# UniBwTAS/continuous_clustering

Hardware: AMD Instinct MI355X
Metric: Mpoints/s clustered (64-beam streams) (higher is better)
Workload: dtype f32

## Files before the change

continuous_clustering_amd/csrc/cc_engine.hip:

```cpp
#include <hip/hip_runtime.h>

#include <algorithm>
#include <chrono>
#include <cstdlib>
#include <cmath>
#include <cstdio>
#include <cstring>
#include <functional>
#include <limits>
#include <mutex>
#include <string>
#include <vector>

#include "cc_kernels.h"

#ifndef CC_LWAVE_MAX_STREAMS
#define CC_LWAVE_MAX_STREAMS 256
#endif

using namespace ccd;

struct cc_engine
{
    int device{0};
// ... 1483 lines not shown
    c->is_single_threaded = 0;
    c->sensor_is_clockwise = 1;
    c->num_columns = 1700;
    c->supplement_inclination_angle_for_nan_cells = 1;
    c->max_slope = 0.2f;
    c->first_ring_as_ground_max_allowed_z_diff = 0.4f;
    c->first_ring_as_ground_min_allowed_z_diff = -0.4f;
    c->last_ground_point_slope_higher_than = -0.1f;
    c->last_ground_point_distance_smaller_than = 5.f;
    c->ground_because_close_to_last_certain_ground_max_z_diff = 0.4f;
    c->ground_because_close_to_last_certain_ground_max_dist_diff = 2.0f;
    c->obstacle_because_next_certain_obstacle_max_dist_diff = 0.3f;
    c->use_terrain = 0;
    c->terrain_max_allowed_z_diff = 0.4f;
    c->fog_filtering_enabled = 0;
    c->fog_filtering_intensity_below = 2;
    c->fog_filtering_distance_below = 18.f;
    c->fog_filtering_inclination_above = -0.06f;
    c->max_distance = 0.7f;
    c->max_steps_in_row = 20;
    c->max_steps_in_column = 20;
    c->stop_after_association_enabled = 1;
    c->stop_after_association_min_steps = 1;
    c->ignore_points_in_chessboard_pattern = 1;
    c->ignore_points_with_too_big_inclination_angle_diff = 1;
    c->use_last_point_for_cluster_stamp = 0;
    c->cluster_point_trees_every_nth_column = 1;
}

void cc_config_kitti(cc_config* c)
{
    cc_config_default(c);
    c->is_single_threaded = 1;
    c->num_columns = 2200;
    c->ignore_points_in_chessboard_pattern = 0;
    c->max_distance = 0.5f;
    c->height_ref_to_maximum_ = 0.5f;
    c->height_ref_to_ground_ = -1.7f;
    c->length_ref_to_front_end_ = 3.f;
    c->length_ref_to_rear_end_ = -3.f;
    c->width_ref_to_left_mirror_ = 1.5f;
    c->width_ref_to_right_mirror_ = -1.5f;
}

const char* cc_version(void)
{
    return "continuous_clustering_amd 0.1 gfx950";
}

int cc_engine_create(cc_engine** out, int device, int num_streams, int num_rows, const cc_config* cfg)
{
    if (!out)
        return CC_ERR_INVALID_ARGUMENT;
    *out = nullptr;
    int rc = validate(nullptr, cfg, num_rows, num_streams);
    if (rc)
        return rc;
    int ndev = 0;
    if (hipGetDeviceCount(&ndev) != hipSuccess || ndev <= 0 || device < 0 || device >= ndev)
        return CC_ERR_NO_DEVICE;
    cc_engine* e = new cc_engine();
    e->device = device;
    StreamSet set;
    if (hipSetDevice(device) != hipSuccess || !acquire_stream_set(device, &set))
    {
        delete e;
        return CC_ERR_HIP;
    }
    e->stream = set.s[0], e->stream2 = set.s[1], e->stream3 = set.s[2], e->stream4 = set.s[3], e->stream5 = set.s[4], e->stream6 = set.s[5];
    for_each_event(e, [](hipEvent_t& ev) { (void) hipEventCreateWithFlags(&ev, hipEventDisableTiming); });
    e->cfg = *cfg;
    e->widest_steps_in_row = cfg->max_steps_in_row;
    e->g.num_streams = num_streams;
    e->g.tree_capacity = 1 << 15;
    e->g.record_events = num_streams == 1 ? 1 : 0;
    e->g.mirror_fields = e->g.record_events;
    e->g.link_capacity = num_streams <= 8 ? (1 << 20) : 8192;
    fill_geometry(e, num_rows);
    e->g.event_capacity = e->g.record_events ? 3 * (e->g.limit_columns + e->g.num_columns) + 4096 : 1;
    e->pending_events.resize(num_streams);
    e->pending_links.resize(num_streams);
    e->state_cache.resize(num_streams);
    e->state_cached.assign(num_streams, 0);
    (void) hipFuncSetAttribute((const void*) cck::k_seg_scan, hipFuncAttributeMaxDynamicSharedMemorySize, 160 * 1024);
    (void) hipFuncSetAttribute((const void*) cck::k_insert2<1>, hipFuncAttributeMaxDynamicSharedMemorySize, 160 * 1024);
    (void) hipFuncSetAttribute((const void*) cck::k_small_front, hipFuncAttributeMaxDynamicSharedMemorySize, 160 * 1024);
    (void) hipFuncSetAttribute((const void*) cck::k_small_all, hipFuncAttributeMaxDynamicSharedMemorySize, 96 * 1024);
    (void) hipFuncSetAttribute((const void*) cck::k_insert2<2>, hipFuncAttributeMaxDynamicSharedMemorySize, 160 * 1024);
    (void) hipFuncSetAttribute((const void*) (cck::k_insert_par<1, cck::IP_WAVES>), hipFuncAttributeMaxDynamicSharedMemorySize, 120 * 1024);
    (void) hipFuncSetAttribute((const void*) (cck::k_insert_par<1, 2 * cck::IP_WAVES>), hipFuncAttributeMaxDynamicSharedMemorySize, 120 * 1024);
    rc = allocate(e);
    if (rc == CC_OK)
        rc = alloc_pinned(e, &e->h_par_left, 8 * sizeof(int), PIN_ENGINE);
    {
        const char* hp = std::getenv("CC_HOST_PROF");
        e->host_prof = hp && hp[0] == '1';
    }
    if (rc == CC_OK)
        rc = alloc_pinned(e, &e->h_bail_count, 4 * sizeof(int), PIN_ENGINE);
    if (rc == CC_OK)
        e->h_bail_count[0] = e->h_bail_count[1] = e->h_bail_count[2] = e->h_bail_count[3] = 0;
    if (rc == CC_OK)
        rc = alloc_pinned(e, &e->h_remaining, sizeof(int), PIN_ENGINE);
    if (rc == CC_OK)
    {
        *e->h_remaining = 0;
        rc = reset_state(e, false);
    }
    if (rc != CC_OK)
    {
        fprintf(stderr, "cc_engine_create: %s\n", e->error.c_str());
        free_all(e);
        free_pinned(e, PIN_ENGINE);
        give_back_streams(e);
        delete e;
        return rc;
    }
    for (const char* name : {"small_front", "seg_small_max", "fuse_front"})
    {
        if (!getenv("CC_ENABLE_ENV_OPTS"))
            break;
        std::string key = std::string("CC_OPT_") + name;
        for (auto& ch : key)
            ch = (char) toupper((unsigned char) ch);
        if (const char* v = getenv(key.c_str()))
            (void) cc_engine_set_option(e, name, atoll(v));
    }
    *out = e;
    return CC_OK;
}

void cc_engine_destroy(cc_engine* e)
{
    if (!e)
        return;
    (void) hipSetDevice(e->device);
    (void) stop_resident(e);
    if (e->host_prof && e->hp_calls > 0)
        fprintf(stderr, "[cc host_prof] gated calls %lld: entry->launch_batch %.1f us, launch_batch->gate %.1f us, gate wait %.1f us, gate->return %.1f us (per call)\n",
                e->hp_calls, e->hp_entry / e->hp_calls * 1e6, e->hp_pre / e->hp_calls * 1e6, e->hp_gate / e->hp_calls * 1e6, e->hp_post / e->hp_calls * 1e6);
    (void) for_each_stream(e, [](hipStream_t s) -> int
    {
        (void) hipStreamSynchronize(s);
        return CC_OK;
    });
    e->deferred_tail = nullptr;
    e->lazy_pending = false;
    destroy_small_graphs(e);
    free_all(e);
    free_pinned(e, PIN_ENGINE);
    for_each_event(e, [](hipEvent_t& ev) { (void) hipEventDestroy(ev); });
    for (hipEvent_t ev : e->pev_pool)
        (void) hipEventDestroy(ev);
    for (hipEvent_t ev : e->ev_pool)
        (void) hipEventDestroy(ev);
    give_back_streams(e);
    delete e;
}

int cc_engine_set_config(cc_engine* e, const cc_config* cfg)
{
    if (!e || !cfg)
        return CC_ERR_INVALID_ARGUMENT;
    destroy_small_graphs(e);
    int rc = validate(e, cfg, e->g.num_rows, e->g.num_streams);
    if (rc)
        return rc;
// ... 1105 lines not shown
```

continuous_clustering_amd/csrc/cc_k_segment.h:

```cpp
#pragma once


template<int RPL>
__device__ __forceinline__ void table_scan_tiles(const SP& p, const int R, const int ntiles, const int lane)
{
    float carry[RPL];
#pragma unroll
    for (int k = 0; k < RPL; k++)
    {
        const int row = k * 64 + lane;
        carry[k] = row < R ? p.curtab[row] : 0.f;
    }
    constexpr int U = 8;
    for (int t0 = 0; t0 < ntiles; t0 += U)
    {
        float v[U][RPL];
#pragma unroll
        for (int u = 0; u < U; u++)
#pragma unroll
            for (int k = 0; k < RPL; k++)
            {
                const int row = k * 64 + lane;
                v[u][k] = (row < R && t0 + u < ntiles) ? p.tabc[(size_t) (t0 + u) * R + row] : __builtin_nanf("");
            }
// ... 104 lines not shown
    for (int i = 0; i < 3; i++)
        for (int j = 0; j < 3; j++)
            ir[i * 3 + j] = T[j * 4 + i];
    for (int i = 0; i < 3; i++)
        it[i] = ((-ir[i * 3 + 0]) * T[3] + (-ir[i * 3 + 1]) * T[7]) + (-ir[i * 3 + 2]) * T[11];
    double* o = out + ((size_t) sl * (size_t) n + (size_t) f) * EGO_STRIDE;
    for (int i = 0; i < 3; i++)
    {
        for (int j = 0; j < 3; j++)
            o[i * 3 + j] = (A[i * 4 + 0] * ir[0 * 3 + j] + A[i * 4 + 1] * ir[1 * 3 + j]) + A[i * 4 + 2] * ir[2 * 3 + j];
        o[9 + i] = ((A[i * 4 + 0] * it[0] + A[i * 4 + 1] * it[1]) + A[i * 4 + 2] * it[2]) + A[i * 4 + 3];
    }
    auto gram_dev = [](const double* m, const int stride) -> double
    {
        double dev = 0.;
        for (int a = 0; a < 3; a++)
            for (int b = 0; b < 3; b++)
            {
                double d = 0.;
                for (int k = 0; k < 3; k++)
                    d += m[k * stride + a] * m[k * stride + b];
                d -= a == b ? 1. : 0.;
                dev += d * d;
            }
        return __builtin_sqrt(dev);
    };
    const double dev_t = gram_dev(T, 4), dev_a = gram_dev(A, 4);
    auto mx2 = [](const float a, const float b) -> double
    {
        const double x = a, y = b;
        return x * x > y * y ? x * x : y * y;
    };
    const double box = __builtin_sqrt(mx2(cfg.length_ref_to_front_end_, cfg.length_ref_to_rear_end_) + mx2(cfg.width_ref_to_left_mirror_, cfg.width_ref_to_right_mirror_) +
                                      mx2(cfg.height_ref_to_maximum_, cfg.height_ref_to_ground_));
    const double at = __builtin_sqrt((A[3] * A[3] + A[7] * A[7]) + A[11] * A[11]);
    double skip = __builtin_inf();
    if (dev_t < 0.5 && dev_a < 0.5 && box == box && at == at)
    {
        const double sigma = __builtin_sqrt((1. - dev_t) * (1. - dev_a));
        const double delta = 2.4e-7 * ((__builtin_fabs(T[3]) + __builtin_fabs(T[7])) + __builtin_fabs(T[11])) + 1e-6;
        const double r = ((box + at) / sigma + delta) * 1.00001;
        const double r2 = r * r * 1.00001;
        float r2f = (float) r2;
        if ((double) r2f < r2)
            r2f = __builtin_bit_cast(float, __builtin_bit_cast(int, r2f) + 1);
        skip = r2f == r2f ? (double) r2f : __builtin_inf();
    }
    o[12] = skip;
}

__global__ __launch_bounds__(256) void k_ego(const StreamState* __restrict__ states, int first_stream, cc_config cfg, const double* __restrict__ poses,
                                             long long n, long long n_total, long long fbase, double* __restrict__ out)
{
    const long long f = (long long) blockIdx.x * 256 + threadIdx.x;
    if (f < n)
        ego_record(states, first_stream, cfg, poses, n, n_total, fbase, out, (int) blockIdx.y, f);
}


template<int RPL>
__global__ __launch_bounds__(64) void k_seg_pre(Geometry g, cc_config cfg, Planes P, StreamState* states, int first_stream, int slot,
                                                const double* __restrict__ poses, long long n_total, long long fbase,
                                                const double* __restrict__ ego, long long n_batch)
{
    const int sl = blockIdx.x;
    const int s = first_stream + sl;
    StreamState* st = &states[s];
    const long long seg_begin = st->batch[slot].seg_begin, seg_end = st->batch[slot].seg_end;
    if (seg_begin < 0 || seg_begin >= seg_end)
        return;
    if (st->batch[slot].fused)
        return;
    if (!st->has_robot_tf)
    {
        if (blockIdx.y == 0 && lane_id() == 0)
            raise_error(st, CC_ERR_NO_ROBOT_TRANSFORM, seg_begin, 0);
        return;
    }
    const SP p = stream_ptrs(P, g, s);
    const int R = g.num_rows, RC = g.ring_cols;
    const int lane = lane_id();

    const long long total = seg_end - seg_begin;
    const long long chunk_len = (total + SEGPRE_BLOCKS - 1) / SEGPRE_BLOCKS;
    const long long c_lo = seg_begin + chunk_len * (long long) blockIdx.y, c_hi = (c_lo + chunk_len < seg_end ? c_lo + chunk_len : seg_end);
    if (c_lo >= c_hi)
        return;
    const int NC = g.num_columns;
    int lc = (int) (c_lo % RC);
    long long rot = c_lo / NC;
    int cir = (int) (c_lo - rot * NC);
    long long pass = c_lo / RC;
    uint16_t a_tg[RPL];
    uint16_t n_tg[RPL];
    float n_dist[RPL], n_incaz[RPL];
    float4 n_rec[RPL];
    uint8_t n_inten[RPL];
    int n_trig = 0;
    auto load_tags = [&](const long long gcx, const int lcx)
    {
#pragma unroll
        for (int k = 0; k < RPL; k++)
        {
            const int row = k * 64 + lane;
            a_tg[k] = CELL_CLEARED;
            if (row < R && gcx < c_hi)
                a_tg[k] = p.gtag[(size_t) lcx * R + row];
        }
    };
    auto load_cells = [&](const long long gcx, const int lcx, const uint16_t tagx)
    {
#pragma unroll
        for (int k = 0; k < RPL; k++)
        {
            const int row = k * 64 + lane;
            n_dist[k] = n_incaz[k] = 0.f;
            n_inten[k] = 0;
            n_rec[k] = make_float4(__builtin_nanf(""), __builtin_nanf(""), __builtin_nanf(""), __builtin_nanf(""));
            if (row < R && gcx < c_hi)
            {
                const size_t ci = (size_t) lcx * R + row;
                n_dist[k] = p.dist[ci];
                if (n_tg[k] == tagx)
                {
                    n_rec[k] = p.sc_rec[ci];
                    n_incaz[k] = p.incaz[ci];
                    n_inten[k] = p.inten[ci];
                }
            }
        }
        if (gcx < c_hi)
            n_trig = p.trig[lcx];
    };
    load_tags(c_lo, lc);
    CazBase cb = caz_base_of_rotation(rot);
    long long cb_rot = rot;
    for (long long gc = c_lo; gc < c_hi; gc++, pass += (lc + 1 == RC ? 1 : 0), lc = (lc + 1 == RC ? 0 : lc + 1), rot += (cir + 1 == NC ? 1 : 0),
                   cir = (cir + 1 == NC ? 0 : cir + 1))
    {
        const size_t base = (size_t) lc * R;
        if (rot != cb_rot)
        {
            cb = caz_base_of_rotation(rot);
            cb_rot = rot;
        }
        const uint16_t tag = cell_tag(pass);
        {
#pragma unroll
            for (int k = 0; k < RPL; k++)
                n_tg[k] = a_tg[k];
            load_cells(gc, lc, tag);
            load_tags(gc + 1, lc + 1 == RC ? 0 : lc + 1);
        }
        const int trig = uniform_i32(n_trig);
        const double* T = poses + ((size_t) sl * (size_t) n_total + (size_t) fbase + (size_t) trig) * 12;
        const double* E = ego + ((size_t) sl * (size_t) n_batch + (size_t) trig) * EGO_STRIDE;
        const float spx = (float) T[3], spy = (float) T[7], spz = (float) T[11];

        float cx[RPL], cy[RPL], cz[RPL], dist[RPL], incl[RPL];
        bool empty_cell[RPL], overrun = false;
        int overrun_row = -1;
        long long overrun_gcol = -1;
#pragma unroll
        for (int k = 0; k < RPL; k++)
        {
            const int row = k * 64 + lane;
            dist[k] = incl[k] = __builtin_nanf("");
// ... 10 lines not shown
                }
                empty_cell[k] = tg != tag;
                dist[k] = n_dist[k];
                cx[k] = n_rec[k].x;
                cy[k] = n_rec[k].y;
                cz[k] = n_rec[k].z;
                incl[k] = n_rec[k].w;
            }
        }
        if (__any(overrun))
        {
            const int worst = -wave_min_i32(-overrun_row);
            if (overrun_row == worst)
            {
                atomicMin((unsigned long long*) &st->overrun_col, (unsigned long long) gc);
                raise_error(st, CC_ERR_RING_OVERRUN, overrun_gcol, gc);
            }
            continue;
        }
        float x2[RPL], uz[RPL], w[RPL];
        int flags[RPL];
        seg_pre_cells<RPL>(cfg, R, lane, cx, cy, cz, dist, incl, n_inten, spx, spy, spz, E, x2, uz, w, flags);
        int kpos = 0x7fffffff, kneg = 0x7fffffff;
        bool any_empty = false;
#pragma unroll
        for (int k = 0; k < RPL; k++)
        {
            const int row = k * 64 + lane;
            if (row >= R)
                continue;
            const size_t ci = base + row;
            if (empty_cell[k])
                p.gtag[ci] = tag;
            if (flags[k] & SG_NAN)
                any_empty = true;
            else
                caz_key(n_incaz[k], kpos, kneg);
            p.sg_x2[ci] = x2[k];
            p.sg_uz[ci] = uz[k];
            p.sg_w[ci] = w[k];
            p.sg_flags[ci] = (uint8_t) flags[k];
        }
        const double min_az = column_min_caz(cb, kpos, kneg, any_empty, gc, g.az_width);
        if (lane == 0)
        {
            p.colg[lc] = gc;
            p.colminaz[lc] = min_az;
        }
    }
}

#ifndef CC_SEGSCAN_MIN_WAVES_PER_SIMD
#define CC_SEGSCAN_MIN_WAVES_PER_SIMD 2
#endif
constexpr int SEG_X2_RING = 16;
constexpr int SEG_CH = 16;
constexpr int SEG_FEW = 4;
__host__ __device__ inline int seg_pitch_f(int R)
{
    (void) R;
    return SEG_X2_RING + 1;
}
__host__ __device__ inline int seg_pitch_b(int R)
{
    return ((R + 3) & ~3) + 4;
}
__host__ __device__ inline bool seg_tiled(int R)
{
    return R >= SEG_CH && (R % SEG_CH) == 0;
}
__host__ inline size_t seg_scan_lds_bytes(int R)
{
    const size_t f = seg_tiled(R) ? (size_t) 4 * 64 * SEG_CH * 4 : (size_t) 64 * seg_pitch_f(R) * 4;
    return f + (size_t) 64 * seg_pitch_b(R);
}

enum
{
    SG_G_UNKNOWN = 0, SG_G_GROUND = 1, SG_G_OBSTACLE = 2, SG_G_EGO = 3, SG_G_FOG = 4,
    SG_D_WHITE = 0, SG_D_GRAY = 1, SG_D_ORANGE = 2, SG_D_GREEN = 3, SG_D_YELLOWGREEN = 4, SG_D_YELLOW = 5, SG_D_RED = 6, SG_D_DARKRED = 7,
    SG_D_VIOLET = 8, SG_D_LIGHTGRAY = 9
};

__global__ __launch_bounds__(64, CC_SEGSCAN_MIN_WAVES_PER_SIMD) void k_seg_scan(Geometry g, cc_config cfg, Planes P, StreamState* states, int first_stream, int slot)
{
    const int s = first_stream + blockIdx.x;
    StreamState* st = &states[s];
    const long long seg_begin = st->batch[slot].seg_begin, seg_end = st->batch[slot].seg_end;
    if (seg_begin < 0 || st->error != 0)
        return;
    const long long tile0 = seg_begin + (long long) blockIdx.y * 64;
    if (tile0 >= seg_end)
        return;
    const int ncols = (int) (seg_end - tile0 < 64 ? seg_end - tile0 : 64);
    const SP p = stream_ptrs(P, g, s);
    const int R = g.num_rows, RC = g.ring_cols;
    const int lane = lane_id();
    const int PF = seg_pitch_f(R), PB = seg_pitch_b(R);
    const bool tiled = seg_tiled(R);
    extern __shared__ __attribute__((aligned(16))) unsigned char smem[];
    float* l_x2 = (float*) smem;
    unsigned char* l_out = (unsigned char*) (l_x2 + (tiled ? 4 * 64 * SEG_CH : 64 * PF));

    const int lc0 = (int) (tile0 % RC);
    {
        const bool active = lane < ncols;
        const long long gc = tile0 + lane;
        int lcl = lc0 + lane;
        lcl = lcl >= RC ? lcl - RC : lcl;
        const float* gx = p.sg_x2 + (size_t) lcl * R;
        const float* gz = p.sg_uz + (size_t) lcl * R;
        const float* gw = p.sg_w + (size_t) lcl * R;
        const unsigned char* gf = p.sg_flags + (size_t) lcl * R;
        float4* g_rec = p.sc_rec + (size_t) lcl * R;
        float* g_incl = p.incl + (size_t) lcl * R;
        const float* tab_in = p.tabc + (size_t) blockIdx.y * R;
        unsigned char* oo = l_out + lane * PB;
        const float height_sensor_to_ground = -(float) st->robot_from_sensor[11] + cfg.height_ref_to_ground_;
        const bool chess_odd = cfg.ignore_points_in_chessboard_pattern && (gc & 1);
        const bool chess_even = cfg.ignore_points_in_chessboard_pattern && !(gc & 1);
        bool first_obstacle_detected = false, first_point_found = false;
        float lg2x = 0.f, lgz = height_sensor_to_ground;
        float pv2x = 0.f, pvz = 0.f;
        unsigned char previous_label = 0;
        auto row_step = [&](const int row, const int f, const float cur2x, const float cur2y, auto&& x2_below)
        {
            const bool valid = (f & (SG_NAN | SG_FOG | SG_EGO)) == 0;
            const bool first = valid & !first_point_found;
            const bool normal = valid & first_point_found;
            const bool ign = ((f & (SG_TOO_CLOSE | SG_INCL_IGNORE)) != 0) | ((row & 1) ? chess_even : chess_odd);
            const float h = cur2y - height_sensor_to_ground;
            const bool first_ground = (h > cfg.first_ring_as_ground_min_allowed_z_diff) & (h < cfg.first_ring_as_ground_max_allowed_z_diff);
            const float p2cx = cur2x - pv2x, p2cy = cur2y - pvz;
            const float slope_to_prev = p2cy / p2cx;
            const bool flat_prev = (ccm::absf(slope_to_prev) < cfg.max_slope) & (p2cx > 0) & ((cfg.use_terrain == 0) | (p2cx < 5));
            const float l2cx = cur2x - lg2x, l2cy = cur2y - lgz;
            const float slope_to_lg = l2cy / l2cx;
            const bool flat_lg = (ccm::absf(slope_to_lg) < cfg.max_slope) & (l2cx > 0);
            const bool no_terrain = cfg.use_terrain == 0;
            const bool green = !first_obstacle_detected & flat_prev;
            const bool yellowgreen = !green & no_terrain & first_obstacle_detected & flat_prev & flat_lg;
            const bool yellow = !green & !yellowgreen & no_terrain &
                                (ccm::absf(l2cx) < cfg.ground_because_close_to_last_certain_ground_max_dist_diff) &
                                (ccm::absf(l2cy) < cfg.ground_because_close_to_last_certain_ground_max_z_diff);
            const bool ground_n = green | yellowgreen | yellow;
            const unsigned d_n = green ? (unsigned) SG_D_GREEN : (yellowgreen ? (unsigned) SG_D_YELLOWGREEN : (yellow ? (unsigned) SG_D_YELLOW : (unsigned) SG_D_RED));
            const unsigned g_n = ground_n ? (unsigned) SG_G_GROUND : (unsigned) SG_G_OBSTACLE;
            const unsigned d_f = first_ground ? (unsigned) SG_D_GRAY : (unsigned) SG_D_ORANGE;
            const unsigned g_f = first_ground ? (unsigned) SG_G_GROUND : (unsigned) SG_G_OBSTACLE;
            unsigned g = first ? g_f : g_n, d = first ? d_f : d_n;
            g = (f & SG_EGO) ? (unsigned) SG_G_EGO : g;
            d = (f & SG_EGO) ? (unsigned) SG_D_VIOLET : d;
            g = (f & SG_FOG) ? (unsigned) SG_G_FOG : g;
            d = (f & SG_FOG) ? (unsigned) SG_D_LIGHTGRAY : d;
            g = (f & SG_NAN) ? (unsigned) SG_G_UNKNOWN : g;
            d = (f & SG_NAN) ? (unsigned) SG_D_WHITE : d;
            const bool red = normal & !ground_n;
            if (__any(red))
            {
                int below = row + 1;
                bool go = red & (below < R);
                while (__any(go))
                {
                    const int bi = go ? below : row + 1 < R ? row + 1 : row;
                    const unsigned bo = oo[bi];
                    const unsigned bg = bo & 7u, bd = (bo >> 3) & 15u;
                    const float xb = x2_below(bi, go);
                    const bool is_ground = bg == (unsigned) SG_G_GROUND;
                    const bool cont = go & ((bd == (unsigned) SG_D_YELLOW) |
                                            (is_ground & (ccm::absf(cur2x - xb) < cfg.obstacle_because_next_certain_obstacle_max_dist_diff)));
                    if (cont & is_ground)
                        oo[bi] = (unsigned char) ((bo & 0x80u) | SG_G_OBSTACLE | (SG_D_DARKRED << 3));
                    below += cont ? 1 : 0;
                    go = cont & (below < R);
                }
            }
            first_obstacle_detected = first ? !first_ground : (first_obstacle_detected | red);
            const bool keep_as_ground = normal & (green | yellowgreen) & (slope_to_prev > cfg.last_ground_point_slope_higher_than) &
                                        (ccm::absf(p2cx) < cfg.last_ground_point_distance_smaller_than) & (previous_label != SG_D_YELLOW);
            const bool new_lg = (first & first_ground) | keep_as_ground;
            lg2x = new_lg ? cur2x : lg2x;
            lgz = new_lg ? cur2y : lgz;
            pv2x = valid ? cur2x : pv2x;
            pvz = valid ? cur2y : pvz;
            previous_label = valid ? (unsigned char) d : previous_label;
            first_point_found |= valid;
            oo[row] = (unsigned char) (g | (d << 3) | ((valid & ign) ? 0x80u : 0u));
        };
        const unsigned long long le_mask = lane == 63 ? ~0ull : ((2ull << lane) - 1ull);
        const bool supplement = cfg.supplement_inclination_angle_for_nan_cells != 0;
        const bool step_filter = cfg.ignore_points_with_too_big_inclination_angle_diff != 0;
        float supp_below = __builtin_nanf("");
        bool below_nan = false;
        auto row_all = [&](const int row, const int f, const float cur2x, const float cur2y, const float wv, const float carry, auto&& x2_below,
                           auto&& stash) -> bool
        {
            const bool own = !(f & (SG_NAN | SG_PENDING));
            const unsigned long long m = __ballot(own) & le_mask;
            const int src = m ? 63 - __clzll((long long) m) : lane;
// ... 222 lines not shown
                    {
                        const int rr = b + u;
                        nx[u] = rr >= 0 ? gx[rr] : 0.f;
                        nz[u] = rr >= 0 ? gz[rr] : 0.f;
                        nw[u] = rr >= 0 ? gw[rr] : 0.f;
                        const unsigned f = rr >= 0 ? gf[rr] : (unsigned) SG_NAN;
                        if (u < 4)
                            nf0 |= f << (8 * u);
                        else
                            nf1 |= f << (8 * (u - 4));
                    }
                }
            };
            int b = R - 8;
            load_chunk(b);
            for (; b > -8; b -= 8)
            {
                float x8[8], z8[8], w8[8];
#pragma unroll
                for (int u = 0; u < 8; u++)
                {
                    x8[u] = nx[u];
                    z8[u] = nz[u];
                    w8[u] = nw[u];
                }
                const unsigned f0 = nf0, f1 = nf1;
                if (b - 8 > -8)
                    load_chunk(b - 8);
#pragma unroll
                for (int u = 0; u < 8; u++)
                    if (b + u >= 0)
                        x2[(b + u) & (SEG_X2_RING - 1)] = x8[u];
                auto x2_below = [&](const int below, const bool wanted) -> float
                {
                    float v = x2[below & (SEG_X2_RING - 1)];
                    const bool deep = wanted & (below >= b + SEG_X2_RING);
                    if (__any(deep))
                        if (deep)
                            v = gx[below];
                    return v;
                };
#pragma unroll
                for (int u = 7; u >= 0; u--)
                {
                    const int row = b + u;
                    if (row < 0)
                        break;
                    float tab_u = 0.f;
                    const bool pend = row_all(row, (int) (((u < 4 ? f0 : f1) >> (8 * (u & 3))) & 0xffu), x8[u], z8[u], w8[u], tab_in[row], x2_below,
                                              [&](const float tab) { tab_u = tab; });
                    if (__any(pend))
                        if (pend && ccm::atan2f_exact(cfg.max_distance, w8[u]) < tab_u)
                            oo[row] |= 0x80;
                }
            }
        }
    }
    __syncthreads();
    {
        int lc = lc0;
        for (int c = 0; c < ncols; c++)
        {
            for (int row = lane; row < R; row += 64)
            {
                const size_t ci = (size_t) lc * R + row;
                const unsigned char o = l_out[c * PB + row];
                constexpr unsigned long long GV = (unsigned long long) CC_GP_UNKNOWN | ((unsigned long long) CC_GP_GROUND << 8) |
                                                  ((unsigned long long) CC_GP_OBSTACLE << 16) | ((unsigned long long) CC_GP_EGO_VEHICLE << 24) |
                                                  ((unsigned long long) CC_GP_FOG << 32);
                constexpr unsigned long long DV0 = (unsigned long long) CC_DBG_WHITE | ((unsigned long long) CC_DBG_GRAY << 8) |
                                                   ((unsigned long long) CC_DBG_ORANGE << 16) | ((unsigned long long) CC_DBG_GREEN << 24) |
                                                   ((unsigned long long) CC_DBG_YELLOWGREEN << 32) | ((unsigned long long) CC_DBG_YELLOW << 40) |
                                                   ((unsigned long long) CC_DBG_RED << 48) | ((unsigned long long) CC_DBG_DARKRED << 56);
                constexpr unsigned DV1 = (unsigned) CC_DBG_VIOLET | ((unsigned) CC_DBG_LIGHTGRAY << 8);
                const unsigned dcode = (o >> 3) & 15;
                p.ground[ci] = (unsigned char) (GV >> (8 * (o & 7)));
                p.debug[ci] = (unsigned char) (dcode < 8 ? (DV0 >> (8 * dcode)) : (unsigned long long) (DV1 >> (8 * (dcode - 8))));
                const bool ign = (o & 7) != SG_G_OBSTACLE || (o & 0x80);
                p.ignored[ci] = ign ? 1 : 0;
            }
            lc = lc + 1 == RC ? 0 : lc + 1;
        }
    }
}

__device__ __forceinline__ void seg_small_body(const Geometry& g, const cc_config& cfg, const Planes& P, StreamState* states, int first_stream, int slot,
                                               const double* __restrict__ poses, long long n_total, long long fbase, const double* __restrict__ ego,
                                               long long n_batch, const int sl)
{
    const int s = first_stream + sl;
    StreamState* st = &states[s];
    const int lane = lane_id();
    if (lane == 0)
        st->batch[slot].mode = st->assoc_mode;
    const long long seg_begin = st->batch[slot].seg_begin, seg_end = st->batch[slot].seg_end;
    if (seg_begin < 0 || seg_begin >= seg_end || st->error != 0)
        return;
    if (!st->has_robot_tf)
    {
        if (lane == 0)
            raise_error(st, CC_ERR_NO_ROBOT_TRANSFORM, seg_begin, 0);
        return;
    }
    const SP p = stream_ptrs(P, g, s);
    const int R = g.num_rows, RC = g.ring_cols, NC = g.num_columns;
    const int row = lane;
    const bool inrow = row < R;
    const float height_sensor_to_ground = -(float) st->robot_from_sensor[11] + cfg.height_ref_to_ground_;
    const bool supplement = cfg.supplement_inclination_angle_for_nan_cells != 0;
    const bool step_filter = cfg.ignore_points_with_too_big_inclination_angle_diff != 0;
    const bool no_terrain = cfg.use_terrain == 0;
    const unsigned long long le = lane == 63 ? ~0ull : ((2ull << lane) - 1ull);
    const unsigned long long below = ~le, above = le >> 1;
    float tabrow = inrow ? p.curtab[row] : 0.f;
    int lc = (int) (seg_begin % RC);
    long long rot = seg_begin / NC;
    int cir = (int) (seg_begin - rot * NC);
    long long pass = seg_begin / RC;
    CazBase cb = caz_base_of_rotation(rot);
    for (long long gc = seg_begin; gc < seg_end; gc++)
    {
        const size_t ci = (size_t) lc * R + row;
        const uint16_t tag = cell_tag(pass);
        float cx[1] = {0.f}, cy[1] = {0.f}, cz[1] = {0.f}, dist[1] = {__builtin_nanf("")}, incl[1] = {__builtin_nanf("")};
        uint8_t inten[1] = {0};
        float incaz = 0.f;
        bool empty_cell = false, overrun = false;
        long long overrun_gcol = -1;
        if (inrow)
        {
            const uint16_t tg = p.gtag[ci];
            dist[0] = p.dist[ci];
            if (tg == tag)
            {
                const float4 r4 = p.sc_rec[ci];
                cx[0] = r4.x, cy[0] = r4.y, cz[0] = r4.z, incl[0] = r4.w;
                incaz = p.incaz[ci];
                inten[0] = p.inten[ci];
            }
            else
            {
                empty_cell = true;
                if (tg != CELL_CLEARED)
                {
                    overrun = true;
                    overrun_gcol = gc - (long long) ((((unsigned) tag - (unsigned) tg) & 0x7fffu)) * RC;
                }
            }
        }
        if (__any(overrun))
        {
            const int worst = -wave_min_i32(overrun ? -row : 1);
            if (overrun && row == worst)
            {
                atomicMin((unsigned long long*) &st->overrun_col, (unsigned long long) gc);
                raise_error(st, CC_ERR_RING_OVERRUN, overrun_gcol, gc);
            }
            break;
        }
        const int trig = uniform_i32(p.trig[lc]);
        const double* T = poses + ((size_t) sl * (size_t) n_total + (size_t) fbase + (size_t) trig) * 12;
        const double* E = ego + ((size_t) sl * (size_t) n_batch + (size_t) trig) * EGO_STRIDE;
        float x2a[1], uza[1], wa[1];
        int fla[1];
        seg_pre_cells<1>(cfg, R, lane, cx, cy, cz, dist, incl, inten, (float) T[3], (float) T[7], (float) T[11], E, x2a, uza, wa, fla);
        const int f = fla[0];
// ... 159 lines not shown
```

continuous_clustering_amd/csrc/cc_launch.h:

```cpp
#define CC_TARGS(...) __VA_ARGS__
#define CC_LAUNCH_RPL_T(kern_, targs_, rpl_, grid_, block_, lds_, st_, ...)               \
    do                                                                                     \
    {                                                                                      \
        if ((rpl_) == 1)                                                                   \
            hipLaunchKernelGGL((kern_<1 targs_>), grid_, block_, lds_, st_, __VA_ARGS__); \
        else                                                                               \
            hipLaunchKernelGGL((kern_<2 targs_>), grid_, block_, lds_, st_, __VA_ARGS__); \
    } while (0)
#define CC_LAUNCH_RPL(kern_, rpl_, ...) CC_LAUNCH_RPL_T(kern_, , rpl_, __VA_ARGS__)
#define CC_LAUNCH_RPL_MIRROR(kern_, rpl_, mirror_, ...)                   \
    do                                                                    \
    {                                                                     \
        if (mirror_)                                                      \
            CC_LAUNCH_RPL_T(kern_, CC_TARGS(, true), rpl_, __VA_ARGS__);  \
        else                                                              \
            CC_LAUNCH_RPL_T(kern_, CC_TARGS(, false), rpl_, __VA_ARGS__); \
    } while (0)

struct BatchPass
{
    hipStream_t si, sb, sc, sa, sp;
    int slot, first_stream, count;
    int64_t n;
    const float* d_xyz;
    const uint8_t* d_int;
    const double* d_pose;
    bool first_pass, prep_done;
    int rpl;
    long long cur_ntotal, cur_f0;
    int prep_buf;
    Planes Pt;
    double* d_ego;
    int *gate_left, *gate_h_left;
    bool par, gate, gate2, may_defer, lazy, fuse;
    uint64_t rel_seq;
    bool mark;
    hipEvent_t ev[NEV];
};

struct TailArgs
{
    bool fallbacks;
    bool need_segpre;
    bool pre_done;
    bool hp_gated;
    std::chrono::steady_clock::time_point hp_t1;
};

#define CC_MARK(which_, st_) \
    if (bp.mark)             \
        CC_HIP_CHECK(e, hipEventRecord(bp.ev[which_], st_));

static void launch_ego(cc_engine* e, const BatchPass& bp, hipStream_t st)
{
    hipLaunchKernelGGL(cck::k_ego, dim3((unsigned) ((bp.n + 255) / 256), (unsigned) bp.count), dim3(256), 0, st, (const StreamState*) e->d_states, bp.first_stream,
                       e->cfg, bp.d_pose, (long long) bp.n, bp.cur_ntotal, bp.cur_f0, bp.d_ego);
}

static int enqueue_fused_insertion(cc_engine* e, const BatchPass& bp, const int* prev_left, const bool lazy)
{
    const Geometry& g = e->g;
    const hipStream_t si = bp.si;
    const int count = bp.count;
    const double* ego_in = bp.fuse ? (const double*) bp.d_ego : (const double*) nullptr;
    int* left = bp.gate ? bp.gate_left : (int*) nullptr;
    const bool gate_zeroed = bp.gate && bp.first_pass && si != bp.sb && !use_small_front(e, count, bp.n, true);
    if (bp.fuse)
    {
        launch_ego(e, bp, si);
    }
    if (bp.gate && !gate_zeroed)
        CC_HIP_CHECK(e, hipMemsetAsync(left, 0, 2 * sizeof(int), si));
    if (count <= e->insert_wide_max_streams)
    {
        const int nb = e->insert_split_blocks > 0 ? e->insert_split_blocks
                                                  : (count <= 24 ? 8 : (count <= 32 ? 6 : (count <= 40 ? 4 : (count <= 64 ? 3 : (count <= 96 ? 2 : 1)))));
        hipLaunchKernelGGL((cck::k_insert_par<1, 2 * cck::IP_WAVES>), dim3(count, nb), dim3(128 * cck::IP_WAVES), 0, si, g, e->cfg, bp.Pt, e->d_states,
                           bp.first_stream, bp.d_xyz, bp.d_int, bp.d_pose, (long long) bp.n, bp.cur_ntotal, bp.cur_f0, bp.slot, left, ego_in, prev_left);
        if (nb > 1)
            hipLaunchKernelGGL(cck::k_insert_par_fin<1>, dim3(count), dim3(256), 0, si, g, bp.Pt, e->d_states, bp.first_stream, bp.d_xyz, (long long) bp.n,
                               bp.cur_ntotal, bp.cur_f0, bp.slot, left, bp.fuse ? 1 : 0, prev_left);
    }
    else
        hipLaunchKernelGGL((cck::k_insert_par<1, cck::IP_WAVES>), dim3(count), dim3(64 * cck::IP_WAVES), 0, si, g, e->cfg, bp.Pt, e->d_states,
                           bp.first_stream, bp.d_xyz, bp.d_int, bp.d_pose, (long long) bp.n, bp.cur_ntotal, bp.cur_f0, bp.slot, left, ego_in, prev_left);
    if (bp.gate)
    {
        hipLaunchKernelGGL(k_gate_out, dim3(1), dim3(64), 0, si, (const int*) left, (const int*) e->d_bail_count, (const int*) e->d_remaining, bp.gate_h_left,
                           e->h_bail_count, lazy ? e->h_remaining : (int*) nullptr);
    }
    if (lazy)
    {
        CC_HIP_CHECK(e, hipEventRecord(e->ev_ins[bp.slot], si));
        CC_HIP_CHECK(e, hipEventRecord(e->ev_gate[bp.slot], si));
    }
    return CC_OK;
}

static int wait_host_gate(cc_engine* e, const BatchPass& bp, const std::chrono::steady_clock::time_point hp_t0, TailArgs& ta)
{
    const auto hp1 = std::chrono::steady_clock::now();
    CC_HIP_CHECK(e, hipStreamSynchronize(bp.si));
    ta.hp_t1 = std::chrono::steady_clock::now();
    if (e->host_prof)
    {
        e->hp_pre += std::chrono::duration<double>(hp1 - hp_t0).count();
        e->hp_gate += std::chrono::duration<double>(ta.hp_t1 - hp1).count();
        ta.hp_gated = true;
    }
    return CC_OK;
}

static int enqueue_insert_multi(cc_engine* e, const BatchPass& bp, const std::chrono::steady_clock::time_point hp_t0, TailArgs& ta)
{
    const hipStream_t si = bp.si;
    if (bp.gate2)
        CC_HIP_CHECK(e, hipMemsetAsync(e->d_par_left, 0, sizeof(int), si));
    int* left2 = bp.gate2 ? e->d_par_left : (int*) nullptr;
    CC_LAUNCH_RPL(cck::k_insert_multi, bp.rpl, dim3(bp.count), dim3(64 * cck::IM_WAVES), 0, si, e->g, e->cfg, e->P, e->d_states, bp.first_stream, bp.d_xyz,
                  bp.d_int, bp.d_pose, (long long) bp.n, bp.cur_ntotal, bp.cur_f0, bp.slot, left2);
    if (bp.gate2)
    {
        CC_HIP_CHECK(e, hipMemcpyAsync(e->h_par_left, e->d_par_left, sizeof(int), hipMemcpyDeviceToHost, si));
        if (e->h_bail_count)
            CC_HIP_CHECK(e, hipMemcpyAsync(e->h_bail_count, e->d_bail_count, 3 * sizeof(int), hipMemcpyDeviceToHost, si));
        int rcw = wait_host_gate(e, bp, hp_t0, ta);
        if (rcw)
            return rcw;
        ta.fallbacks = *e->h_par_left != 0;
    }
    return CC_OK;
}

static int enqueue_insert_serial(cc_engine* e, const BatchPass& bp, const TailArgs& ta)
{
    const hipStream_t si = bp.si, sp = bp.sp;
    if (bp.first_pass && !bp.prep_done && ta.fallbacks)
    {
        int rcp = launch_prep(e, bp.count, bp.n, bp.d_xyz, bp.d_pose, bp.prep_buf, sp, bp.cur_ntotal, bp.cur_f0, bp.par, bp.first_stream);
        if (rcp)
            return rcp;
    }
    if (!ta.pre_done)
        CC_MARK(EV_PREP, sp);
    if (sp != si)
    {
        CC_HIP_CHECK(e, hipEventRecord(e->ev_prep[bp.slot], sp));
        CC_HIP_CHECK(e, hipStreamWaitEvent(si, e->ev_prep[bp.slot], 0));
    }
    if (ta.fallbacks)
    {
        const Planes Pins = planes_with_prep(e, bp.prep_buf);
        CC_LAUNCH_RPL(cck::k_insert2, bp.rpl, dim3(bp.count), dim3(128), cck::insert2_lds_bytes(e->g.num_rows), si, e->g, e->cfg, Pins, e->d_states,
                      bp.first_stream, bp.slot, bp.d_int, (long long) bp.n, e->d_remaining, bp.cur_ntotal, bp.cur_f0);
    }
    if (!ta.pre_done)
        CC_MARK(EV_INSERT, si);
    if (!ta.pre_done && !e->capture_mirror.state)
        CC_HIP_CHECK(e, hipMemcpyAsync(e->h_remaining, e->d_remaining, sizeof(int), hipMemcpyDeviceToHost, si));
    return CC_OK;
}

static int launch_segmentation(cc_engine* e, const BatchPass& bp, const TailArgs& ta)
{
    const Geometry& g = e->g;
    const hipStream_t si = bp.si, sb = bp.sb, sc = bp.sc;
    const bool seg_small = !bp.par && bp.rpl == 1 && bp.first_pass && bp.n <= e->seg_small_max;
    const bool need_segpre = ta.need_segpre && !seg_small;
    const bool table_early = si != sb;
    if (table_early && need_segpre)
        CC_LAUNCH_RPL(cck::k_table, bp.rpl, dim3(bp.count), dim3(64 * cck::TABLE_WAVES), 0, si, g, bp.Pt, e->d_states, bp.first_stream, bp.slot);
    if (si != sb)
    {
        if (!ta.pre_done)
            CC_HIP_CHECK(e, hipEventRecord(e->ev_ins[bp.slot], si));
        CC_HIP_CHECK(e, hipStreamWaitEvent(sb, e->ev_ins[bp.slot], 0));
    }
    CC_MARK(EV_CHAIN2, sb);
    if (!table_early && need_segpre)
        CC_LAUNCH_RPL(cck::k_table, bp.rpl, dim3(bp.count), dim3(64 * cck::TABLE_WAVES), 0, sb, g, bp.Pt, e->d_states, bp.first_stream, bp.slot);
    if (need_segpre)
    {
        if (!bp.fuse)
            launch_ego(e, bp, sb);
        CC_LAUNCH_RPL(cck::k_seg_pre, bp.rpl, dim3((unsigned) bp.count, cck::SEGPRE_BLOCKS), dim3(64), 0, sb, g, e->cfg, bp.Pt, e->d_states, bp.first_stream,
                      bp.slot, bp.d_pose, bp.cur_ntotal, bp.cur_f0, (const double*) bp.d_ego, (long long) bp.n);
    }
    if (seg_small)
    {
        launch_ego(e, bp, sb);
        hipLaunchKernelGGL(cck::k_seg_small, dim3((unsigned) bp.count), dim3(64), 0, sb, g, e->cfg, e->P, e->d_states, bp.first_stream, bp.slot, bp.d_pose,
                           bp.cur_ntotal, bp.cur_f0, (const double*) bp.d_ego, (long long) bp.n);
    }
    else
    {
        const long long max_cols = std::min<long long>((long long) g.limit_columns + g.num_columns, (long long) g.ring_cols);
        const dim3 seg_grid((unsigned) bp.count, (unsigned) ((max_cols + 63) / 64));
        hipLaunchKernelGGL(cck::k_seg_scan, seg_grid, dim3(64), cck::seg_scan_lds_bytes(g.num_rows), sb, g, e->cfg, bp.Pt, e->d_states, bp.first_stream,
                           bp.slot);
    }
    if (sc != sb)
    {
        CC_HIP_CHECK(e, hipEventRecord(e->ev_segscan[bp.slot], sb));
        CC_HIP_CHECK(e, hipStreamWaitEvent(sc, e->ev_segscan[bp.slot], 0));
    }
    CC_MARK(EV_SEGMENT, sc);
    return CC_OK;
}

struct AssocPlan
{
    bool batch_assoc;
    int rounds;
    int blocks;
    bool lwave;
    int scan_stores_fin;
};

static AssocPlan plan_association(cc_engine* e, const BatchPass& bp, const bool small_front)
{
    const int count = bp.count;
    bool batch_assoc = e->assoc_batch && e->cfg.cluster_point_trees_every_nth_column == 1;
    if (batch_assoc && e->assoc_rounds == 0 && e->h_bail_count && !e->capturing && count >= 8)
    {
        const int seen_now = *e->h_bail_count;
        if (e->chronic_skip > 0)
        {
            e->chronic_skip--;
            e->bail_seen = seen_now;
            batch_assoc = false;
            if (e->chronic_skip == 0)
                e->bail_cooldown = e->bail_cooldown_batches > 2 ? e->bail_cooldown_batches : 2;
        }
        else if ((seen_now - e->chronic_seen) * 4 >= count && e->chronic_probe)
            e->chronic_skip = 8;
        e->chronic_probe = batch_assoc;
        e->chronic_seen = seen_now;
    }
    int adaptive_rounds = 1;
    if (e->assoc_rounds == 0 && e->h_bail_count && !e->capturing)
    {
        const int seen = *e->h_bail_count;
        if (seen != e->bail_seen)
        {
            e->bail_seen = seen;
            e->bail_cooldown = e->bail_cooldown_batches;
        }
        if (e->bail_cooldown > 0)
        {
            e->bail_cooldown--;
            adaptive_rounds = 3;
        }
    }
    AssocPlan plan{batch_assoc, batch_assoc ? (e->assoc_rounds > 0 ? e->assoc_rounds : adaptive_rounds) : 1, count, false, 0};
    const bool idle_net = batch_assoc && e->assoc_rounds == 0 && adaptive_rounds == 1;
    if (idle_net && !e->capturing && e->assoc_sweep_blocks < count)
        plan.blocks = e->assoc_sweep_blocks;
    plan.lwave = e->assoc_waves == 4 || (e->assoc_waves_auto && count <= CC_LWAVE_MAX_STREAMS);
    plan.scan_stores_fin = (!small_front && !idle_net) ? 1 : 0;
    if (e->scan_store_fin >= 0 && !small_front)
        plan.scan_stores_fin = e->scan_store_fin;
    return plan;
}

struct ScanChoice
{
    bool packed, split;
};

static ScanChoice choose_scan(cc_engine* e, const BatchPass& bp)
{
    const int rpl = bp.rpl, count = bp.count;
    const bool packed_default = e->scan_packed == 1 || (e->scan_packed < 0 && (rpl > 1 || count > 192));
    if (e->g.mirror_fields || e->scan_split == 0)
        return {packed_default, false};
    if (e->scan_split == 1 || !e->h_bail_count || e->capturing)
        return {packed_default, packed_default && e->scan_split == 1};
    const unsigned vis = (unsigned) e->h_bail_count[1], cols = (unsigned) e->h_bail_count[2];
    const unsigned dc = cols - e->split_cols_seen, dv = vis - e->split_rec_seen;
    if (dc >= 1024u)
    {
        const double rate = (double) dv / ((double) dc * (double) rpl);
        e->split_on = e->split_on ? rate > 20.0 : rate > 40.0;
        e->split_cols_seen = cols, e->split_rec_seen = vis;
    }
    const bool probe = (e->split_probe++ & 31u) == 0u;
    const bool promote = !packed_default && e->scan_packed < 0 && rpl == 1 && count >= 48;
    const bool split = (e->split_on || probe) && (packed_default || promote);
    return {packed_default || (promote && split), split};
}

static int launch_scan(cc_engine* e, const BatchPass& bp, const ScanChoice scan, const Geometry& gs)
{
    const Geometry& g = e->g;
    const hipStream_t sc = bp.sc;
    const dim3 scan_grid((unsigned) bp.count, cck::SCAN_BLOCKS);
    if (scan.packed && scan.split)
    {
        const dim3 long_grid((unsigned) bp.count, cck::SCAN_LONG_BLOCKS), epi_grid((unsigned) bp.count, cck::SCAN_EPI_BLOCKS);
        CC_LAUNCH_RPL_T(cck::k_scan2, CC_TARGS(, false, true), bp.rpl, scan_grid, dim3(64), 0, sc, gs, e->cfg, e->P, e->d_states, bp.first_stream, bp.slot);
        CC_LAUNCH_RPL(cck::k_scan2_long, bp.rpl, long_grid, dim3(64), 0, sc, g, e->cfg, e->P, e->d_states, bp.first_stream, bp.slot, e->d_bail_count);
        CC_LAUNCH_RPL(cck::k_scan2_epi, bp.rpl, epi_grid, dim3(64), 0, sc, g, e->cfg, e->P, e->d_states, bp.first_stream, bp.slot, e->d_bail_count);
    }
    else if (scan.packed)
        CC_LAUNCH_RPL_MIRROR(cck::k_scan2, bp.rpl, g.mirror_fields, scan_grid, dim3(64), 0, sc, gs, e->cfg, e->P, e->d_states, bp.first_stream, bp.slot);
    else
        CC_LAUNCH_RPL_MIRROR(cck::k_scan, bp.rpl, g.mirror_fields, scan_grid, dim3(64), 0, sc, gs, e->cfg, e->P, e->d_states, bp.first_stream, bp.slot);
    CC_MARK(EV_SCAN, sc);
    if (sc != bp.sa)
    {
        CC_HIP_CHECK(e, hipEventRecord(e->ev_seg[bp.slot], sc));
        CC_HIP_CHECK(e, hipStreamWaitEvent(bp.sa, e->ev_seg[bp.slot], 0));
    }
    return CC_OK;
}

static void launch_assocb(cc_engine* e, const BatchPass& bp)
{
    CC_LAUNCH_RPL(cck::k_assocb, bp.rpl, dim3(bp.count), dim3(cck::AB_THREADS), 0, bp.sa, e->g, e->cfg, e->P, e->d_states, bp.first_stream, bp.slot,
                  e->d_bail_count);
}

static int launch_association(cc_engine* e, const BatchPass& bp, const AssocPlan& plan, const Geometry& gs)
{
    const hipStream_t sa = bp.sa;
    const int count = bp.count;
    CC_MARK(EV_CHAIN3, sa);
    bool marked7 = false;
    bool global_done = false;
    if (e->assoc_waves >= 2 && e->cfg.cluster_point_trees_every_nth_column == 1)
    {
        const dim3 block(plan.lwave ? cck::A3_THREADS : 192);
        for (int r = 0; r < plan.rounds; r++)
        {
            if (plan.batch_assoc)
            {
                launch_assocb(e, bp);
                if (r == 0)
                {
                    CC_MARK(EV_ASSOC_LDS, sa);
                    marked7 = true;
                }
            }
            const int limited = r + 1 < plan.rounds ? 1 : 0;
            CC_LAUNCH_RPL(cck::k_assoc3, bp.rpl, dim3(plan.blocks), block, 0, sa, gs, e->cfg, e->P, e->d_states, bp.first_stream, bp.slot, limited, count, 1);
            global_done = limited == 0;
        }
    }
    else
    {
        if (plan.batch_assoc)
        {
            launch_assocb(e, bp);
            CC_MARK(EV_ASSOC_LDS, sa);
            marked7 = true;
        }
        CC_LAUNCH_RPL(cck::k_assoc_lds, bp.rpl, dim3(count), dim3(64), 0, sa, gs, e->cfg, e->P, e->d_states, bp.first_stream, bp.slot);
    }
    if (!marked7)
        CC_MARK(EV_ASSOC_LDS, sa);
    if (!global_done)
        CC_LAUNCH_RPL(cck::k_associate, bp.rpl, dim3(count), dim3(64), 0, sa, e->g, e->cfg, e->P, e->d_states, bp.first_stream, bp.slot);
    CC_MARK(EV_ASSOC_GLOBAL, sa);
    return CC_OK;
}

static int publish_and_release(cc_engine* e, const BatchPass& bp, const TailArgs& ta, const bool batch_assoc, const bool with_publish)
{
    const hipStream_t si = bp.si, sa = bp.sa;
    if (batch_assoc && !bp.gate && !bp.gate2 && e->h_bail_count && !e->capturing)
        CC_HIP_CHECK(e, hipMemcpyAsync(e->h_bail_count, e->d_bail_count, 3 * sizeof(int), hipMemcpyDeviceToHost, sa));
    const bool ids = e->g.publish_ids != 0;
    hipStream_t spub = (si != sa && ids) ? e->stream6 : sa;
    if (spub != sa)
    {
        CC_HIP_CHECK(e, hipEventRecord(e->ev_pubrdy[bp.slot], sa));
        CC_HIP_CHECK(e, hipStreamWaitEvent(spub, e->ev_pubrdy[bp.slot], 0));
    }
    if (with_publish && (ids || e->capture_mirror.state))
        hipLaunchKernelGGL(cck::k_publish, ids ? dim3((unsigned) bp.count, cck::PUBLISH_BLOCKS) : dim3(1), dim3(64), 0, spub, e->g, e->P, e->d_states,
                           bp.first_stream, bp.slot, e->capture_mirror);
    CC_MARK(EV_PUBLISH, spub);
// ... 206 lines not shown
```

Before: 19690.

## Size segment and scan grids to batch work, add strided seg_scan path

Grid y-dimensions for seg_pre, scan, scan_long and scan_epi are now capped by the number of items in the batch instead of fixed block counts. seg_pre computes its chunk length from gridDim.y. For small batches, seg_scan launches a templated strided variant where each block loops over several 64-column tiles, with an LDS fence between iterations. The aim is to avoid launching many blocks that exit immediately and to cut scheduling overhead for small increments. In exchange, small batches get less parallelism per launch, and the other kernels must be correct for grid-stride or early-exit use with fewer blocks.

```diff
diff --git a/continuous_clustering_amd/csrc/cc_engine.hip b/continuous_clustering_amd/csrc/cc_engine.hip
--- a/continuous_clustering_amd/csrc/cc_engine.hip
+++ b/continuous_clustering_amd/csrc/cc_engine.hip
@@ -1589,7 +1589,8 @@
     e->pending_links.resize(num_streams);
     e->state_cache.resize(num_streams);
     e->state_cached.assign(num_streams, 0);
-    (void) hipFuncSetAttribute((const void*) cck::k_seg_scan, hipFuncAttributeMaxDynamicSharedMemorySize, 160 * 1024);
+    (void) hipFuncSetAttribute((const void*) cck::k_seg_scan<false>, hipFuncAttributeMaxDynamicSharedMemorySize, 160 * 1024);
+    (void) hipFuncSetAttribute((const void*) cck::k_seg_scan<true>, hipFuncAttributeMaxDynamicSharedMemorySize, 160 * 1024);
     (void) hipFuncSetAttribute((const void*) cck::k_insert2<1>, hipFuncAttributeMaxDynamicSharedMemorySize, 160 * 1024);
     (void) hipFuncSetAttribute((const void*) cck::k_small_front, hipFuncAttributeMaxDynamicSharedMemorySize, 160 * 1024);
     (void) hipFuncSetAttribute((const void*) cck::k_small_all, hipFuncAttributeMaxDynamicSharedMemorySize, 96 * 1024);
diff --git a/continuous_clustering_amd/csrc/cc_k_segment.h b/continuous_clustering_amd/csrc/cc_k_segment.h
--- a/continuous_clustering_amd/csrc/cc_k_segment.h
+++ b/continuous_clustering_amd/csrc/cc_k_segment.h
@@ -210,7 +210,7 @@
     const int lane = lane_id();
 
     const long long total = seg_end - seg_begin;
-    const long long chunk_len = (total + SEGPRE_BLOCKS - 1) / SEGPRE_BLOCKS;
+    const long long chunk_len = (total + (long long) gridDim.y - 1) / (long long) gridDim.y;
     const long long c_lo = seg_begin + chunk_len * (long long) blockIdx.y, c_hi = (c_lo + chunk_len < seg_end ? c_lo + chunk_len : seg_end);
     if (c_lo >= c_hi)
         return;
@@ -387,20 +387,21 @@
     SG_D_VIOLET = 8, SG_D_LIGHTGRAY = 9
 };
 
-__global__ __launch_bounds__(64, CC_SEGSCAN_MIN_WAVES_PER_SIMD) void k_seg_scan(Geometry g, cc_config cfg, Planes P, StreamState* states, int first_stream, int slot)
-{
-    const int s = first_stream + blockIdx.x;
-    StreamState* st = &states[s];
+template<bool STRIDED>
+__device__ __forceinline__ bool seg_scan_tile(const Geometry& g, const cc_config& cfg, const Planes& P, const StreamState* states, int s, const int slot, int tile)
+{
+    int R = g.num_rows, RC = g.ring_cols, lane = lane_id();
+    if constexpr (STRIDED)
+        asm volatile("" : "+s"(s), "+s"(tile), "+s"(R), "+s"(RC), "+v"(lane));
+    const StreamState* st = &states[s];
     const long long seg_begin = st->batch[slot].seg_begin, seg_end = st->batch[slot].seg_end;
     if (seg_begin < 0 || st->error != 0)
-        return;
-    const long long tile0 = seg_begin + (long long) blockIdx.y * 64;
+        return false;
+    const long long tile0 = seg_begin + (long long) tile * 64;
     if (tile0 >= seg_end)
-        return;
+        return false;
     const int ncols = (int) (seg_end - tile0 < 64 ? seg_end - tile0 : 64);
     const SP p = stream_ptrs(P, g, s);
-    const int R = g.num_rows, RC = g.ring_cols;
-    const int lane = lane_id();
     const int PF = seg_pitch_f(R), PB = seg_pitch_b(R);
     const bool tiled = seg_tiled(R);
     extern __shared__ __attribute__((aligned(16))) unsigned char smem[];
@@ -419,7 +420,7 @@
         const unsigned char* gf = p.sg_flags + (size_t) lcl * R;
         float4* g_rec = p.sc_rec + (size_t) lcl * R;
         float* g_incl = p.incl + (size_t) lcl * R;
-        const float* tab_in = p.tabc + (size_t) blockIdx.y * R;
+        const float* tab_in = p.tabc + (size_t) tile * R;
         unsigned char* oo = l_out + lane * PB;
         const float height_sensor_to_ground = -(float) st->robot_from_sensor[11] + cfg.height_ref_to_ground_;
         const bool chess_odd = cfg.ignore_points_in_chessboard_pattern && (gc & 1);
@@ -808,6 +809,18 @@
             lc = lc + 1 == RC ? 0 : lc + 1;
         }
     }
+    return true;
+}
+
+template<bool STRIDED>
+__global__ __launch_bounds__(64, CC_SEGSCAN_MIN_WAVES_PER_SIMD) void k_seg_scan(Geometry g, cc_config cfg, Planes P, StreamState* states, int first_stream, int slot)
+{
+    const int s = first_stream + blockIdx.x;
+    if constexpr (!STRIDED)
+        seg_scan_tile<false>(g, cfg, P, states, s, slot, (int) blockIdx.y);
+    else
+        for (int tile = blockIdx.y; seg_scan_tile<true>(g, cfg, P, states, s, slot, tile); tile += gridDim.y)
+            wave_lds_fence();
 }
 
 __device__ __forceinline__ void seg_small_body(const Geometry& g, const cc_config& cfg, const Planes& P, StreamState* states, int first_stream, int slot,
diff --git a/continuous_clustering_amd/csrc/cc_launch.h b/continuous_clustering_amd/csrc/cc_launch.h
--- a/continuous_clustering_amd/csrc/cc_launch.h
+++ b/continuous_clustering_amd/csrc/cc_launch.h
@@ -51,6 +51,11 @@
     if (bp.mark)             \
         CC_HIP_CHECK(e, hipEventRecord(bp.ev[which_], st_));
 
+static unsigned batch_blocks(const long long items, const long long bound)
+{
+    return (unsigned) std::min<long long>(bound, std::max<long long>(1, items + 1));
+}
+
 static void launch_ego(cc_engine* e, const BatchPass& bp, hipStream_t st)
 {
     hipLaunchKernelGGL(cck::k_ego, dim3((unsigned) ((bp.n + 255) / 256), (unsigned) bp.count), dim3(256), 0, st, (const StreamState*) e->d_states, bp.first_stream,
@@ -183,7 +188,7 @@
     {
         if (!bp.fuse)
             launch_ego(e, bp, sb);
-        CC_LAUNCH_RPL(cck::k_seg_pre, bp.rpl, dim3((unsigned) bp.count, cck::SEGPRE_BLOCKS), dim3(64), 0, sb, g, e->cfg, bp.Pt, e->d_states, bp.first_stream,
+        CC_LAUNCH_RPL(cck::k_seg_pre, bp.rpl, dim3((unsigned) bp.count, batch_blocks(bp.n, cck::SEGPRE_BLOCKS)), dim3(64), 0, sb, g, e->cfg, bp.Pt, e->d_states, bp.first_stream,
                       bp.slot, bp.d_pose, bp.cur_ntotal, bp.cur_f0, (const double*) bp.d_ego, (long long) bp.n);
     }
     if (seg_small)
@@ -195,9 +200,15 @@
     else
     {
         const long long max_cols = std::min<long long>((long long) g.limit_columns + g.num_columns, (long long) g.ring_cols);
-        const dim3 seg_grid((unsigned) bp.count, (unsigned) ((max_cols + 63) / 64));
-        hipLaunchKernelGGL(cck::k_seg_scan, seg_grid, dim3(64), cck::seg_scan_lds_bytes(g.num_rows), sb, g, e->cfg, bp.Pt, e->d_states, bp.first_stream,
-                           bp.slot);
+        const unsigned cover = (unsigned) ((max_cols + 63) / 64);
+        const bool strided = bp.n <= g.num_columns / 2;
+        const dim3 seg_grid((unsigned) bp.count, strided ? batch_blocks((bp.n + 63) / 64, cover) : cover);
+        if (strided)
+            hipLaunchKernelGGL(cck::k_seg_scan<true>, seg_grid, dim3(64), cck::seg_scan_lds_bytes(g.num_rows), sb, g, e->cfg, bp.Pt, e->d_states,
+                               bp.first_stream, bp.slot);
+        else
+            hipLaunchKernelGGL(cck::k_seg_scan<false>, seg_grid, dim3(64), cck::seg_scan_lds_bytes(g.num_rows), sb, g, e->cfg, bp.Pt, e->d_states,
+                               bp.first_stream, bp.slot);
     }
     if (sc != sb)
     {
@@ -294,10 +305,12 @@
 {
     const Geometry& g = e->g;
     const hipStream_t sc = bp.sc;
-    const dim3 scan_grid((unsigned) bp.count, cck::SCAN_BLOCKS);
+    const long long cols_per_trip = scan.packed ? cck::SCAN_TILE_CELLS / (bp.rpl * 64) : 1;
+    const dim3 scan_grid((unsigned) bp.count, batch_blocks((bp.n + cols_per_trip - 1) / cols_per_trip, cck::SCAN_BLOCKS));
     if (scan.packed && scan.split)
     {
-        const dim3 long_grid((unsigned) bp.count, cck::SCAN_LONG_BLOCKS), epi_grid((unsigned) bp.count, cck::SCAN_EPI_BLOCKS);
+        const dim3 long_grid((unsigned) bp.count, batch_blocks(bp.n * bp.rpl, cck::SCAN_LONG_BLOCKS)),
+            epi_grid((unsigned) bp.count, batch_blocks(bp.n, cck::SCAN_EPI_BLOCKS));
         CC_LAUNCH_RPL_T(cck::k_scan2, CC_TARGS(, false, true), bp.rpl, scan_grid, dim3(64), 0, sc, gs, e->cfg, e->P, e->d_states, bp.first_stream, bp.slot);
         CC_LAUNCH_RPL(cck::k_scan2_long, bp.rpl, long_grid, dim3(64), 0, sc, g, e->cfg, e->P, e->d_states, bp.first_stream, bp.slot, e->d_bail_count);
         CC_LAUNCH_RPL(cck::k_scan2_epi, bp.rpl, epi_grid, dim3(64), 0, sc, g, e->cfg, e->P, e->d_states, bp.first_stream, bp.slot, e->d_bail_count);
```

New measurement: 19730 (median of 5 runs). No clear change (+0.2%).
